# slbouknight/accelerated-ray-tracer

Measured on AMD Instinct MI355X. Metric: Mrays/s, 1200x800 random scene @ 500 spp (frame ms in ms_per_step), higher is better.
Workload: dtype f32

## Files before the change

### accelerated-ray-tracer_amd/csrc/rt_abi.hip

```cpp
#include <hip/hip_runtime.h>

#include <algorithm>
#include <cfloat>
#include <utility>
#include <cmath>
#include <functional>
#include <cstdio>
#include <cstring>
#include <string>
#include <vector>

#include "../../include/rt_abi.h"
#include "rt_device.h"
#include "rt_refit_host.h"

namespace {

struct device_info {
    bool ready = false;
    int num_cu = 256;
    size_t lds_per_cu = 160 * 1024;
};
enum { RT_MAX_DEVICES = 16 };
device_info g_devices[RT_MAX_DEVICES];
// ... 2223 lines not shown
            HIPCHK(hipMemcpy((void*)*v.dev, v.host, list_bytes, hipMemcpyHostToDevice));
        }
        HIPCHK(mem.get((void**)&mp.out, list_bytes));
        HIPCHK(hipMemset(mp.out, 0xFF, list_bytes));
    }
    HIPCHK(rt_launch_math_tests(mp, nullptr));
    HIPCHK(hipDeviceSynchronize());
    if (sweep) HIPCHK(hipMemcpy(digests, mp.digests, n_digests * sizeof(unsigned long long), hipMemcpyDeviceToHost));
    else HIPCHK(hipMemcpy(out, mp.out, list_bytes, hipMemcpyDeviceToHost));
    return RT_OK;
}

rt_status rt_debug_cal_cost(rt_scene* s, uint32_t* out, int32_t cap, int32_t* nx, int32_t* ny) {
    if (!s) return invalid("rt_debug_cal_cost: null scene");
    if (!out || !nx || !ny) return invalid("rt_debug_cal_cost: null argument");
    if (cap < 64) return invalid("rt_debug_cal_cost: cap must be at least 64 (the smallest calibration grid is 8 x 8)");
    if (!s->d_cal_cost || s->cal_nx <= 0 || s->cal_ny <= 0) return invalid("rt_debug_cal_cost: the scene kept no calibration costs");
    *nx = s->cal_nx; *ny = s->cal_ny;
    if ((long long)cap < (long long)s->cal_nx * s->cal_ny) return invalid("rt_debug_cal_cost: cap is smaller than the calibration grid (nx and ny are set)");
    RT_TRY(use_device(s->device));
    HIPCHK(hipMemcpy(out, s->d_cal_cost, (size_t)s->cal_nx * s->cal_ny * sizeof(unsigned int), hipMemcpyDeviceToHost));
    return RT_OK;
}

rt_status rt_debug_cost_map(rt_scene* s, uint32_t* out, int64_t cap, int32_t* info4) {
    if (!s) return invalid("rt_debug_cost_map: null scene");
    if (!info4 || (!out && cap != 0)) return invalid("rt_debug_cost_map: null argument");
    RT_TRY(use_device(s->device));
    if (s->frame_pending) RT_TRY(rt_frame_finish(s, nullptr));
    const rt_scene::cost_map_state& cm = s->cost_map;
    const bool have = g_opt.cost_map && cm.valid;
    info4[0] = !have ? 0 : (cm.scene_epoch == s->scene_epoch && cm.opt_epoch == g_opt_epoch ? 1 : 2);
    info4[1] = have ? cm.key.nx : 0; info4[2] = have ? cm.key.local_rows : 0; info4[3] = cm.last_parts;
    if (!have || !out) return RT_OK;
    const long long n = (long long)cm.key.nx * cm.key.local_rows;
    if ((long long)cap < n) return invalid("rt_debug_cost_map: cap is smaller than the map (info is set)");
    HIPCHK(hipMemcpy(out, cm.d, (size_t)n * sizeof(unsigned int), hipMemcpyDeviceToHost));
    return RT_OK;
}

rt_status rt_debug_set_cost_map(rt_scene* s, const uint32_t* in, int64_t n) {
    if (!s) return invalid("rt_debug_set_cost_map: null scene");
    if (!in) return invalid("rt_debug_set_cost_map: null argument");
    if (!g_opt.cost_map) return invalid("rt_debug_set_cost_map: option cost_map is 0");
    rt_scene::cost_map_state& cm = s->cost_map;
    if (!cm.have_last_key) return invalid("rt_debug_set_cost_map: the scene has rendered no ranked frame");
    if ((long long)n != (long long)cm.last_key.nx * cm.last_key.local_rows) return invalid("rt_debug_set_cost_map: n is not the last ranked frame's local pixel count");
    RT_TRY(use_device(s->device));
    if (s->frame_pending) RT_TRY(rt_frame_finish(s, nullptr));
    std::vector<unsigned int> words((size_t)n);
    unsigned long long total = 0;
    for (size_t k = 0; k < (size_t)n; ++k) { words[k] = in[k] & 0x7FFFFFFFu; total += words[k]; }
    cm.valid = false;
    RT_TRY(grow(cm.d, cm.capacity, (size_t)n));
    HIPCHK(hipMemcpy(cm.d, words.data(), (size_t)n * sizeof(unsigned int), hipMemcpyHostToDevice));
    cm.key = cm.last_key; cm.scene_epoch = s->scene_epoch; cm.opt_epoch = g_opt_epoch; cm.total = total; cm.valid = true;
    return RT_OK;
}

rt_status rt_debug_rank_info(rt_scene* s, uint32_t* out13) {
    if (!s) return invalid("rt_debug_rank_info: null scene");
    if (!out13) return invalid("rt_debug_rank_info: null argument");
    if (!s->ranked_frame || !s->d_rank) return invalid("rt_debug_rank_info: the scene's last frame was not ranked");
    RT_TRY(use_device(s->device));
    if (s->frame_pending) HIPCHK(hipStreamSynchronize(s->pending_stream));
    HIPCHK(hipMemcpy(out13, s->d_rank, sizeof(rt_rank_info), hipMemcpyDeviceToHost));
    return RT_OK;
}

namespace {
struct main_launch {
    int kernel, lds_mode;
    size_t lds_bytes;
    dim3 grid, block;
    int per_cu_resident;
    bool lean_family;
};
rt_status plan_main_launch(const rt_scene* s, int kernel, size_t n_pixels, rt_frame_params& fp, main_launch& ml) {
    const int g_num_cu = g_devices[s->device].num_cu;
    const size_t g_lds_per_cu = g_devices[s->device].lds_per_cu;
    int lds_mode = g_opt.lds_mode;
    const bool lean_family = s->spheres_only && s->tex_level < 2;
    const size_t budget1 = g_lds_per_cu - 2048;
    if (lds_mode < 0) {
        if (s->node_bytes + s->sphere_bytes <= budget1) lds_mode = 2;
        else if (s->node_bytes <= budget1) lds_mode = 1;
        else lds_mode = 0;
    }
    if (g_opt.lds_mode < 0 && kernel == RT_KERNEL_STAGED && g_opt.scan_nodes > 0 && s->dev.n_nodes <= g_opt.scan_nodes) lds_mode = 4;
    if (lds_mode >= 3 && kernel != RT_KERNEL_STAGED) lds_mode = 2;
    if (kernel == RT_KERNEL_PIXEL) lds_mode = 0;
    size_t lds_bytes = 0;
    if (lds_mode >= 1 && lds_mode <= 3) lds_bytes += s->node_bytes;
    if (lds_mode >= 2 && lds_mode <= 3) lds_bytes += s->sphere_bytes;
    if (lds_mode == 3) lds_bytes += s->shade_bytes;
    if (lds_bytes > budget1) return invalid("requested lds_mode does not fit the CU's LDS");
    dim3 grid, block;
    int per_cu_resident = 1;
    if (kernel == RT_KERNEL_PIXEL) {
        block = dim3(256);
        grid = dim3((fp.work_items + 255u) / 256u);
    } else {
        const bool lean = lean_family;
        const int fam_max_threads = lean ? RT_LEAN_MAX_THREADS : RT_HEAVY_MAX_THREADS;
        const int lds_fit = lds_bytes ? (int)(g_lds_per_cu / (lds_bytes + 512)) : 8;
        int per_cu = g_opt.wg_per_cu > 0 ? g_opt.wg_per_cu : (lean ? 2 : 3);
        int threads = g_opt.threads > 0 ? g_opt.threads : (lean ? 512 : 256);
        if (g_opt.wg_per_cu <= 0 && g_opt.threads <= 0 && lds_fit < per_cu) {
            per_cu = 1; threads = fam_max_threads;
        }
        if (lds_fit < per_cu) per_cu = lds_fit < 1 ? 1 : lds_fit;
        if (threads > fam_max_threads) threads = fam_max_threads;
        if (threads < 64) threads = 64;
        block = dim3((unsigned)threads);
        unsigned want = (unsigned)(g_num_cu * per_cu);
        const unsigned need = (fp.work_items + (unsigned)threads - 1) / (unsigned)threads;
        grid = dim3(want < need ? want : need);
        per_cu_resident = per_cu;
    }
    {
        const double pixels_per_lane = (double)n_pixels / ((double)g_num_cu * (double)per_cu_resident * (double)block.x);
        const bool latency_regime = kernel == RT_KERNEL_STAGED && lean_family && pixels_per_lane < 2.75;
        fp.shade_threshold = g_opt.shade_threshold > 0 ? g_opt.shade_threshold : (latency_regime ? 16 : 32);
        fp.newpath_threshold = g_opt.newpath_threshold > 0 ? g_opt.newpath_threshold : (s->spheres_only ? (latency_regime ? 12 : 24) : 8);
    }
    ml.kernel = kernel; ml.lds_mode = lds_mode; ml.lds_bytes = lds_bytes; ml.grid = grid; ml.block = block; ml.per_cu_resident = per_cu_resident;
    ml.lean_family = lean_family;
    return RT_OK;
}

void stats_of_launch(const rt_scene* s, const main_launch& ml, rt_stats& out) {
    out.kernel_variant = ml.kernel * 1000 + ml.lds_mode * 100 + s->tex_level * 10 + (s->spheres_only ? 1 : 0);
    out.workgroups = (int)ml.grid.x; out.threads_per_group = (int)ml.block.x; out.lds_bytes = (int)ml.lds_bytes;
}

void fill_frame_params(const rt_scene* s, const rt_frame_desc* f, const frame_geometry& g, int ns, rt_frame_params& fp) {
    memset(&fp, 0, sizeof(fp));
    fp.ray_counter = s->d_ray_counter;
    fp.work_counter = s->d_work_counter;
    fp.seed_base = f->seed_base;
    fp.nx = f->nx; fp.ny = f->ny; fp.ns = ns; fp.gamma = f->gamma;
    fp.background[0] = f->background[0]; fp.background[1] = f->background[1]; fp.background[2] = f->background[2];
    fp.use_gradient_bg = f->use_gradient_bg;
    fp.tile_rows = f->tile_rows; fp.tile_first = f->tile_first; fp.tile_stride = f->tile_stride;
    fp.local_rows = g.local_rows;
    fp.tiles_x = g.tiles_x;
    fp.work_items = g.work_items;
    fp.sparse_priority = g_opt.sparse_priority; fp.sparse_eager = g_opt.sparse_eager; fp.semi_priority = g_opt.semi_priority; fp.tier_priority = g_opt.tier_priority;
    fp.steps_per_trip = g_opt.steps_per_trip;
    fp.leaf_threshold = g_opt.leaf_threshold;
    fp.diel_threshold = g_opt.diel_threshold;
    fp.box_threshold = g_opt.box_threshold; fp.medium_threshold = g_opt.medium_threshold;
}

struct tier_room {
    bool fits;
    int lds_scene;
    size_t lds;
    unsigned tail_grid;
};
tier_room plan_tier_room(const rt_scene* s, size_t budget) {
    tier_room r = {false, 0, 0, 0};
    const int ns_ = s->dev.n_slots, nsph = s->dev.n_spheres, nm = s->dev.n_materials, nt = s->dev.n_textures;
    if (s->dev.leaf_lo == nullptr || rt_tier_lds_bytes(ns_, nsph, nm, nt, false) > budget) return r;
    r.fits = true;
    r.lds_scene = rt_tier_lds_bytes(ns_, nsph, nm, nt, true) <= budget ? 1 : 0;
    r.lds = rt_tier_lds_bytes(ns_, nsph, nm, nt, r.lds_scene != 0);
    const bool lean_family = s->spheres_only && s->tex_level < 2;
    const unsigned by_lds = (unsigned)(g_devices[s->device].lds_per_cu / (r.lds + 512));
    const unsigned by_regs = lean_family ? 4u : 3u;
    r.tail_grid = (unsigned)g_devices[s->device].num_cu * (by_lds < by_regs ? by_lds : by_regs);
    if (r.tail_grid < 1u) r.tail_grid = 1u;
    return r;
}
hipError_t launch_tier(const rt_scene* s, const rt_frame_params& fp, dim3 grid, size_t lds, hipStream_t stream) {
    return s->spheres_only ? rt_launch_tier_spheres(s->tex_level, s->dev, fp, grid, lds, stream)
// ... 540 lines not shown
```

### accelerated-ray-tracer_amd/csrc/rt_device.h

```cpp
#pragma once
#include <hip/hip_runtime.h>
#include <stdint.h>

#include "../../include/rt_abi.h"

#define RT_PERSISTENT_THREADS 512
#ifndef RT_LEAN_MIN_WAVES
#define RT_LEAN_MIN_WAVES 4
#endif
#ifndef RT_LEAN_MAX_THREADS
#define RT_LEAN_MAX_THREADS 512
#endif
#define RT_HEAVY_MAX_THREADS 768
#define RT_HEAVY_MIN_WAVES 3

#define RT_TIER_THREADS 256
enum { RT_DIAG_BINS = 192, RT_DIAG_T0_SLOT = 32, RT_DIAG_HIST_SLOT = 33, RT_DIAG_WAVE_SLOT = 33 + 2 * 192 + 7, RT_DIAG_MAX_WAVES = 8192,
       RT_COUNTER_BYTES = (33 + 2 * 192 + 7 + 2 * 8192) * 8 };
enum { RT_KERNEL_PIXEL = 0, RT_KERNEL_STAGED = 3 };

struct rt_pixel_state {
    uint32_t rng[6];
    float col[3];
    uint32_t cost;
};

struct rt_rank_info {
    uint32_t heavy_items;
    uint32_t heavy_threshold;
    uint32_t tier1_items;
    uint32_t tier2_items;
    int32_t tier1_wgs;
    int32_t main_skip_wgs;
    int32_t sparse_wgs;
    int32_t sparse_stride;
    int32_t semi_wgs;
    int32_t semi_stride;
    uint32_t threshold1;
    uint32_t threshold2;
    uint32_t collected;
};

struct rt_rank_params {
    rt_pixel_state* state;
    const unsigned int* tile_cost;
    unsigned int* tile_order;
    const unsigned long long* ray_counter;
    unsigned long long* heavy_list;
    unsigned int* heavy_pixels;
    rt_rank_info* info;
    uint32_t n_pixels, n_tiles, heavy_cap;
    uint32_t max_grid, waves_per_wg, normal_need;
    int32_t sparse_stride;
    int32_t semi_stride;
    int32_t sparse_percent;
    int32_t sparse_work_percent;
    int32_t tier_possible;
    int32_t tier1_pixels;
    int32_t tier1_depth;
    int32_t tier_wgs_cap;
    int32_t tier_waves_per_main_wg;
    int32_t nx, smooth_percent;
    float heavy_factor, sparse_factor, tier1_factor;
};

#define RT_NODE_SKIP(stored) (~(stored))

struct rt_scene_dev {
    const rt_node* nodes;
    const rt_node* nodes_ref;
    const rt_sphere* spheres;
    const rt_quad* quads;
    const rt_box* boxes;
    const rt_instance* instances;
    const rt_medium* media;
    const rt_material* materials;
    const rt_texture* textures;
    const uint8_t* images;
    int32_t n_nodes, n_nodes_ref, n_spheres, n_materials, n_textures;
    float bound[3];
    float bound_pad;
    const float4* leaf_lo;
    const float4* leaf_hi;
    const float* slot_ranges;
    int32_t n_leaves, n_slots;
    int32_t n_media_leaves;
    int32_t media_ord[2];
    rt_camera camera;
};

enum { RT_WC_DEAD = 64,
       RT_WC_PUSHED = 65,
       RT_WC_TAIL_HEAD = 66,
       RT_WORK_COUNTER_BYTES = 512 };
struct rt_frame_params {
    float* fb;
    unsigned long long* ray_counter;
    unsigned int* work_counter;
    unsigned int* pixel_cost;
    unsigned int* node_pass;
    int32_t node_pass_lds;
    float* ray_sample;
    uint32_t ray_sample_cap, ray_sample_stride;
    const unsigned int* tile_order;
    unsigned int* tile_cost;
    rt_pixel_state* state_out;
    const rt_pixel_state* state_in;
    int32_t sample_begin, sample_end;
    const unsigned int* heavy_pixels;
    const rt_rank_info* rank;
    int32_t store_parked;
    int32_t fresh;
    int32_t tier_lds_scene;
    unsigned long long* handoff_queue;
    uint32_t handoff_cap;
    rt_pixel_state* handoff_state;
    int32_t handoff_pixels;
    int32_t handoff_poll_ticks;
    int32_t tail_mode;
    unsigned int* cost_out;
    uint64_t seed_base;
    int32_t nx, ny, ns;
    float gamma;
    float background[3];
    int32_t use_gradient_bg;
    int32_t tile_rows, tile_first, tile_stride;
    int32_t local_rows;
    int32_t tiles_x;
    uint32_t work_items;
    int32_t sparse_eager;
    int32_t sparse_priority;
    int32_t tier_priority;
    int32_t semi_priority;
    int32_t steps_per_trip;
    int32_t shade_threshold;
    int32_t leaf_threshold;
    int32_t box_threshold, medium_threshold;
    int32_t diel_threshold;
    int32_t newpath_threshold;
};

hipError_t rt_launch_rank(const rt_rank_params& rp, hipStream_t st);
struct rt_prior_params {
    rt_pixel_state* state;
    unsigned int* tile_cost;
    unsigned long long* total;
    const unsigned int* cal_cost;
    int32_t cal_nx, cal_ny;
    int32_t nx, ny, local_rows, tiles_x;
// ... 286 lines not shown
```

### accelerated-ray-tracer_amd/csrc/rt_device_funcs.h

```cpp
#pragma once
#include <hip/hip_runtime.h>
#include <float.h>
#include <stdint.h>

#include "../../include/rt_abi.h"
#include "rt_device.h"
#include "rt_xorwow.h"

#define DEV __device__ __forceinline__

namespace {

struct f3 { float x, y, z; };
DEV f3 mk3(float x, float y, float z) { f3 r; r.x = x; r.y = y; r.z = z; return r; }
DEV f3 ld3(const float* p) { return mk3(p[0], p[1], p[2]); }
DEV f3 operator+(f3 a, f3 b) { return mk3(a.x + b.x, a.y + b.y, a.z + b.z); }
DEV f3 operator-(f3 a, f3 b) { return mk3(a.x - b.x, a.y - b.y, a.z - b.z); }
DEV f3 operator*(f3 a, f3 b) { return mk3(a.x * b.x, a.y * b.y, a.z * b.z); }
DEV f3 operator*(float t, f3 v) { return mk3(t * v.x, t * v.y, t * v.z); }
DEV f3 operator-(f3 a) { return mk3(-a.x, -a.y, -a.z); }
DEV f3 sdiv(f3 v, float t) { return mk3(v.x / t, v.y / t, v.z / t); }
DEV float dot(f3 a, f3 b) { return fmaf(a.z, b.z, fmaf(a.x, b.x, a.y * b.y)); }
DEV f3 cross(f3 a, f3 b) { return mk3(fmaf(a.y, b.z, -(a.z * b.y)), -fmaf(a.x, b.z, -(a.z * b.x)), fmaf(a.x, b.y, -(a.y * b.x))); }
DEV float length(f3 v) { return sqrtf(fmaf(v.z, v.z, fmaf(v.x, v.x, v.y * v.y))); }
// ... 454 lines not shown
        out.d = random_in_unit_sphere(g);
        attenuation = (TEX > 0 && m.tex >= 0) ? texture_value<TEX>(sc, m.tex, rec.u, rec.v, rec.p) : ld3(m.albedo);
        return true;
    }
    }
}

DEV Ray camera_get_ray(const rt_camera& c, float s, float t, rt_xorwow& g) {
    f3 p;
    do {
        const float a = rt_xorwow_signed(g);
        const float b = rt_xorwow_signed(g);
        p = mk3(a, b, 0.0f);
    } while (dot(p, p) >= 1.0f);
    const f3 rd = c.lens_radius * p;
    const f3 cu = ld3(c.u), cv = ld3(c.v);
    const f3 offset = fma3(rd.x, cu, rd.y * cv);
    const double tm = fma((double)rt_xorwow_uniform(g), c.time1 - c.time0, c.time0);
    const f3 origin = ld3(c.origin);
    Ray r;
    r.o = origin + offset;
    r.d = (fma3(t, ld3(c.vertical), fma3(s, ld3(c.horizontal), ld3(c.lower_left_corner))) - origin) - offset;
    r.tm = (float)tm;
    return r;
}

DEV float apply_gamma(float c, float gamma) {
    if (gamma == 1.0f) return c;
    const float inv = 1.0f / gamma;
    return cr_pow(fmaxf(c, 0.0f), inv);
}

template <typename P>
DEV f3 miss_color(const P& fp, const Ray& r) {
    f3 bg = mk3(fp.background[0], fp.background[1], fp.background[2]);
    if (fp.use_gradient_bg) {
        const f3 ud = unit_vector(r.d);
        const float t = 0.5f * (ud.y + 1.0f);
        bg = mk3(fmaf(t, 0.5f, 1.0f - t), fmaf(t, 0.7f, 1.0f - t), (1.0f - t) + t);
    }
    return bg;
}

DEV bool work_to_pixel(const rt_frame_params& fp, uint32_t w, int& i, int& lrow) {
    const uint32_t tile = fp.tile_order ? fp.tile_order[w >> 6] : (w >> 6), within = w & 63u;
    const uint32_t tx = tile % (uint32_t)fp.tiles_x, ty = tile / (uint32_t)fp.tiles_x;
    i = (int)(tx * 8u + (within & 7u));
    lrow = (int)(ty * 8u + (within >> 3));
    return i < fp.nx && lrow < fp.local_rows;
}
DEV int local_to_global_row(const rt_frame_params& fp, int lrow) {
    const int t = lrow / fp.tile_rows;
    return (fp.tile_first + t * fp.tile_stride) * fp.tile_rows + (lrow - t * fp.tile_rows);
}

DEV void store_pixel(const rt_frame_params& fp, int i, int lrow, f3 col) {
    const float k = (float)(1.0 / (double)(float)fp.ns);
    col = mk3(col.x * k, col.y * k, col.z * k);
    float* px = fp.fb + ((size_t)lrow * fp.nx + i) * 3;
    px[0] = apply_gamma(col.x, fp.gamma);
    px[1] = apply_gamma(col.y, fp.gamma);
    px[2] = apply_gamma(col.z, fp.gamma);
}

typedef float lds_native_float4 __attribute__((ext_vector_type(4)));
DEV int32_t lds_address(const void* p) { return (int32_t)(uint32_t)(uintptr_t)(const __attribute__((address_space(3))) void*)p; }
DEV float4 lds_load_float4(int32_t address, int which) {
    const lds_native_float4 q = ((const __attribute__((address_space(3))) lds_native_float4*)(uintptr_t)(uint32_t)address)[which];
    return make_float4(q.x, q.y, q.z, q.w);
}
DEV int32_t lds_load_word(int32_t address, int word) { return ((const __attribute__((address_space(3))) int32_t*)(uintptr_t)(uint32_t)address)[word]; }

template <int LDS_MODE, bool WALK_LINKS = false>
DEV SceneView stage_scene(const rt_scene_dev& sd, unsigned char* lds) {
    SceneView v;
    v.nodes = sd.nodes; v.spheres = sd.spheres; v.quads = sd.quads; v.boxes = sd.boxes; v.instances = sd.instances;
    v.media = sd.media; v.materials = sd.materials; v.textures = sd.textures; v.images = sd.images; v.n_nodes = sd.n_nodes;
    if (LDS_MODE >= 1 && LDS_MODE <= 3) {
        float4* dst = reinterpret_cast<float4*>(lds);
        const float4* src = reinterpret_cast<const float4*>(sd.nodes);
        const int n16 = sd.n_nodes * 2;
        if (WALK_LINKS) {
            const int32_t base = lds_address(lds);
            for (int k = threadIdx.x; k < n16; k += blockDim.x) {
                float4 q = src[k];
                const int32_t w = __float_as_int(q.w);
                q.w = __int_as_float(w < 0 ? base + 32 * RT_NODE_SKIP(w) : ~w);
                dst[k] = q;
            }
        } else {
            for (int k = threadIdx.x; k < n16; k += blockDim.x) dst[k] = src[k];
        }
        v.nodes = reinterpret_cast<const rt_node*>(lds);
        if (LDS_MODE >= 2) {
            float4* dst2 = dst + n16;
            const float4* src2 = reinterpret_cast<const float4*>(sd.spheres);
            const int m16 = sd.n_spheres * 2;
            for (int k = threadIdx.x; k < m16; k += blockDim.x) dst2[k] = src2[k];
            v.spheres = reinterpret_cast<const rt_sphere*>(dst2);
            if (LDS_MODE >= 3) {
                float4* dst3 = dst2 + m16;
                const float4* src3 = reinterpret_cast<const float4*>(sd.materials);
                const int q16 = sd.n_materials * 2;
                for (int k = threadIdx.x; k < q16; k += blockDim.x) dst3[k] = src3[k];
                v.materials = reinterpret_cast<const rt_material*>(dst3);
                float4* dst4 = dst3 + q16;
                const float4* src4 = reinterpret_cast<const float4*>(sd.textures);
                const int r16 = sd.n_textures * 4;
                for (int k = threadIdx.x; k < r16; k += blockDim.x) dst4[k] = src4[k];
                v.textures = reinterpret_cast<const rt_texture*>(dst4);
            }
        }
        __syncthreads();
    }
    return v;
}

template <bool SPHERES_ONLY>
DEV bool trace(const SceneView& sc, const Ray& r, HitInfo& best, unsigned int* pass_count = nullptr) {
    const f3 inv = mk3(1.0f / r.d.x, 1.0f / r.d.y, 1.0f / r.d.z);
    const float tmin = 0.001f;
    best.t = FLT_MAX; best.prim = -1; best.inst = -1;
    const float4* nodes4 = reinterpret_cast<const float4*>(sc.nodes);
    int i = 0;
    const int n = sc.n_nodes;
    while (i < n) {
        const float4 a = nodes4[2 * i], b = nodes4[2 * i + 1];
        int next = RT_NODE_SKIP(__float_as_int(a.w));
        if (slab_test(a, b, r.o, inv, tmin, best.t)) {
            if (pass_count) atomicAdd(&pass_count[i], 1u);
            const int32_t prim = __float_as_int(b.w);
            if (prim >= 0) leaf_test<SPHERES_ONLY>(sc, prim, r, tmin, best);
            else next = i + 1;
        }
        i = next;
    }
    return best.prim >= 0;
}

DEV bool inv_is_finite(const f3 inv) {
    return fabsf(inv.x) < INFINITY && fabsf(inv.y) < INFINITY && fabsf(inv.z) < INFINITY;
}

DEV void slab_interval(const float4 lo_skip, const float4 hi_prim, const f3 o, const f3 inv, float tmin, float& t_enter, float& t_exit) {
    float tmax = FLT_MAX;
    float t0 = (lo_skip.x - o.x) * inv.x, t1 = (hi_prim.x - o.x) * inv.x;
    if (inv.x < 0.0f) { const float tmp = t0; t0 = t1; t1 = tmp; }
    tmin = t0 > tmin ? t0 : tmin;
    tmax = t1 < tmax ? t1 : tmax;
    t0 = (lo_skip.y - o.y) * inv.y; t1 = (hi_prim.y - o.y) * inv.y;
    if (inv.y < 0.0f) { const float tmp = t0; t0 = t1; t1 = tmp; }
    tmin = t0 > tmin ? t0 : tmin;
    tmax = t1 < tmax ? t1 : tmax;
    t0 = (lo_skip.z - o.z) * inv.z; t1 = (hi_prim.z - o.z) * inv.z;
    if (inv.z < 0.0f) { const float tmp = t0; t0 = t1; t1 = tmp; }
    tmin = t0 > tmin ? t0 : tmin;
    tmax = t1 < tmax ? t1 : tmax;
    t_enter = tmin; t_exit = tmax;
}

DEV bool lane_not(bool b) { return __builtin_amdgcn_inverse_ballot_w64(~__builtin_amdgcn_ballot_w64(b)); }

DEV bool slab_interval_open(float tmin, float tmax, float x0, float x1, float y0, float y1, float z0, float z1) {
    float lo = __builtin_amdgcn_fmed3f(tmin, x0, x1), hi = __builtin_amdgcn_fmed3f(tmax, x0, x1);
    lo = __builtin_amdgcn_fmed3f(lo, y0, y1); hi = __builtin_amdgcn_fmed3f(hi, y0, y1);
    lo = __builtin_amdgcn_fmed3f(lo, z0, z1); hi = __builtin_amdgcn_fmed3f(hi, z0, z1);
    return !(hi <= lo);
}

DEV bool slab_test_finite(const float4 lo_skip, const float4 hi_prim, const f3 o, const f3 inv, float tmin, float tmax) {
    const float x0 = (lo_skip.x - o.x) * inv.x, x1 = (hi_prim.x - o.x) * inv.x;
    const float y0 = (lo_skip.y - o.y) * inv.y, y1 = (hi_prim.y - o.y) * inv.y;
    const float z0 = (lo_skip.z - o.z) * inv.z, z1 = (hi_prim.z - o.z) * inv.z;
    return slab_interval_open(tmin, tmax, x0, x1, y0, y1, z0, z1);
}

struct LooseRay { f3 clo, chi; };
DEV bool loose_ok(const f3 inv, const f3 o, const float* bound) {
// ... 21 lines not shown
```

### accelerated-ray-tracer_amd/csrc/rt_kernel_staged.h

```cpp
#pragma once
#ifndef RT_STEP_UNROLL
#define RT_STEP_UNROLL 2
#endif
#include "rt_device_funcs.h"
#include "rt_launch.h"

#ifdef RT_DIAG
#define DIAG_ADD(slot, value) do { const unsigned long long v_ = (unsigned long long)(value); if ((threadIdx.x & 63) == 0) diag_local[slot] += v_; } while (0)
#define DIAG_T(slot) do { const unsigned long long n_ = __builtin_readcyclecounter(); diag_time[slot] += n_ - diag_t_last; diag_t_last = n_; } while (0)
#else
#define DIAG_ADD(slot, value) do { } while (0)
#define DIAG_T(slot) do { } while (0)
#endif

template <bool SPHERES_ONLY, int TEX, bool NEED_UV, int LDS_MODE>
__global__ void __launch_bounds__((SPHERES_ONLY && TEX < 2) ? RT_LEAN_MAX_THREADS : RT_HEAVY_MAX_THREADS, (SPHERES_ONLY && TEX < 2) ? RT_LEAN_MIN_WAVES : RT_HEAVY_MIN_WAVES) rt_render_staged_kernel(rt_scene_dev sd, rt_frame_params fp) {
    extern __shared__ __attribute__((aligned(16))) unsigned char lds[];
#ifdef RT_DIAG
    unsigned long long diag_local[16] = {0, 0, 0, 0, 0, 0, 0, 0, 0, 0, 0, 0, 0, 0, 0, 0};
    unsigned long long diag_time[8] = {0, 0, 0, 0, 0, 0, 0, 0};
    unsigned long long diag_shade_cycles = 0;
    unsigned long long diag_t_last = 0;
    const unsigned long long diag_t_start = __builtin_amdgcn_s_memrealtime();
    if ((threadIdx.x & 63) == 0) atomicMin(fp.ray_counter + RT_DIAG_T0_SLOT, diag_t_start);
    unsigned long long diag_fetch_t = 0ull, diag_done_t = 0ull;
    unsigned int diag_last_px = 0u, diag_last_src = 0u;
#endif
    constexpr bool SCAN = LDS_MODE == 4;
    rt_rank_info rk;
    rk.heavy_items = 0u; rk.heavy_threshold = 0xFFFFFFFFu; rk.tier1_items = 0u; rk.tier2_items = 0u;
    rk.tier1_wgs = 0; rk.main_skip_wgs = 0; rk.sparse_wgs = 0; rk.sparse_stride = 1; rk.semi_wgs = 0; rk.semi_stride = 1;
    if (fp.rank) {
        const rt_rank_info* q = fp.rank;
        rk.heavy_items = q->heavy_items; rk.heavy_threshold = q->heavy_threshold; rk.tier1_items = q->tier1_items;
        rk.tier2_items = q->tier2_items; rk.semi_wgs = q->semi_wgs; rk.semi_stride = q->semi_stride;
        rk.main_skip_wgs = q->main_skip_wgs; rk.sparse_wgs = q->sparse_wgs; rk.sparse_stride = q->sparse_stride;
    }
    const int wg = (int)blockIdx.x - rk.main_skip_wgs;
    if (wg < 0) return;
    constexpr bool ADDR = LDS_MODE >= 1 && LDS_MODE <= 3;
    const SceneView sc = stage_scene<LDS_MODE, ADDR>(sd, lds);
    const float4* nodes4 = reinterpret_cast<const float4*>(sc.nodes);
    const int n_nodes = sc.n_nodes;
    const int root = ADDR ? lds_address(lds) : 0;
    const int limit = ADDR ? __builtin_amdgcn_readfirstlane(root + 32 * n_nodes) : n_nodes;
    const int ST_DONE = limit, ST_NEWPATH = limit + 1, ST_DIEL = limit + 2, ST_SETUP = limit + 3, ST_DEAD = limit + 4;
    auto node_lo = [&](int at) -> float4 { return ADDR ? lds_load_float4(at, 0) : nodes4[2 * at]; };
    auto node_hi = [&](int at) -> float4 { return ADDR ? lds_load_float4(at, 1) : nodes4[2 * at + 1]; };
    auto leaf_prim = [](const float4 hi) -> int32_t { return ADDR ? ~__float_as_int(hi.w) : __float_as_int(hi.w); };
    const float tmin = 0.001f;

    rt_xorwow g = {0, 0, 0, 0, 0, 0};
    int px_i = 0, px_lrow = 0, px_j = 0, sample = 0, bounce = 0;
    f3 col = mk3(0, 0, 0), throughput = mk3(1, 1, 1), radiance = mk3(0, 0, 0);
    Ray cur; cur.o = mk3(0, 0, 0); cur.d = mk3(0, 0, 1); cur.tm = 0.f;
    f3 inv = mk3(1, 1, 1);
    HitInfo best; best.t = FLT_MAX; best.prim = -1; best.inst = -1;
    int node = ST_NEWPATH;
    int32_t parked = -1;
    int32_t pend = -1;
    float cur_a = 1.f;
    bool have_pixel = false, first = true, finite_inv = true;
    bool tier3_open = true;
    bool leave = false;
    unsigned int wave_dead = 0;
    unsigned long long last_poll = 0ull;
    bool dry_seen = false;
    const uint32_t total_lanes = (uint32_t)((int)gridDim.x - rk.main_skip_wgs) * blockDim.x;
    unsigned int rays = 0, rays_at_pixel_start = 0;
    bool sparse = wg < rk.sparse_wgs;
    bool semi = !sparse && wg < rk.sparse_wgs + rk.semi_wgs;
#ifdef RT_DIAG
    const bool diag_was_sparse = sparse;
#endif
    if (semi && fp.semi_priority > 0) {
        if (fp.semi_priority == 1) __builtin_amdgcn_s_setprio(1);
        else if (fp.semi_priority == 2) __builtin_amdgcn_s_setprio(2);
        else __builtin_amdgcn_s_setprio(3);
    }
    if (sparse && fp.sparse_priority > 0) {
        if (fp.sparse_priority == 1) __builtin_amdgcn_s_setprio(1);
        else if (fp.sparse_priority == 2) __builtin_amdgcn_s_setprio(2);
        else __builtin_amdgcn_s_setprio(3);
    }

#ifdef RT_DIAG
    diag_t_last = __builtin_readcyclecounter();
#endif
    for (;;) {
        DIAG_ADD(0, 1);
        DIAG_T(7);
        if (SCAN) {
            const bool scanning = (unsigned)node < (unsigned)n_nodes;
            if (__ballot(scanning) != 0ull) {
                const bool ref_form = __ballot(scanning && !finite_inv) != 0ull;
                int resume = 0;
                for (int k = 0; k < n_nodes; ++k) {
                    const float4 a = uniform_load(nodes4 + 2 * k), b = uniform_load(nodes4 + 2 * k + 1);
                    const int32_t prim = __builtin_amdgcn_readfirstlane(__float_as_int(b.w));
                    const int skip = RT_NODE_SKIP(__builtin_amdgcn_readfirstlane(__float_as_int(a.w)));
                    const bool active = scanning && k >= resume;
                    DIAG_ADD(1, 1); DIAG_ADD(2, __popcll(__ballot(active)));
                    const bool pass = active && (ref_form ? slab_test(a, b, cur.o, inv, tmin, best.t) : slab_test_finite(a, b, cur.o, inv, tmin, best.t));
                    if (prim < 0) {
                        if (active && !pass) resume = skip;
                        DIAG_T(0);
                    } else if (__ballot(pass) != 0ull) {
                        DIAG_T(0);
                        DIAG_ADD(3, 1); DIAG_ADD(4, __popcll(__ballot(pass)));
                        if (pass) leaf_test<SPHERES_ONLY, true>(sc, prim, cur, tmin, best);
                        DIAG_T(1);
                    }
                }
                if (scanning) node = ST_DONE;
            }
        } else {
        if (__ballot(!finite_inv && (unsigned)node < (unsigned)limit) == 0ull) {
            const int trip_pairs = ((sparse ? 2 * fp.steps_per_trip : fp.steps_per_trip) + RT_STEP_UNROLL - 1) / RT_STEP_UNROLL;
            const LooseRay lr = loose_setup(inv, cur.o, sd.bound);
            for (int pair = 0; pair < trip_pairs; ++pair) {
                if (__ballot((unsigned)node < (unsigned)limit) == 0ull) break;
#pragma unroll
                for (int half = 0; half < RT_STEP_UNROLL; ++half) {
                    DIAG_ADD(1, 1); DIAG_ADD(2, __popcll(__ballot((unsigned)node < (unsigned)limit)));
                    if ((unsigned)node < (unsigned)limit) {
                        const float4 a = node_lo(node), b = node_hi(node);
                        const bool pass = slab_test_loose(a, b, inv, lr, tmin, best.t);
                        if (ADDR) {
                            const int32_t link = __float_as_int(b.w), skip = __float_as_int(a.w);
                            const bool is_leaf = link < 0, noted = pend >= 0;
                            const bool inner = lane_not(is_leaf), clear = lane_not(noted);
                            const bool at_leaf = pass && is_leaf;
                            const bool stop = at_leaf && noted;
                            pend = (at_leaf && clear) ? node : pend;
                            parked = stop ? node : parked;
                            node = (pass && (inner || noted)) ? link : skip;
                        } else {
                            const int32_t link = __float_as_int(b.w), nskip = __float_as_int(a.w);
                            const bool is_leaf = link >= 0, noted = pend >= 0;
                            const bool inner = lane_not(is_leaf), clear = lane_not(noted);
                            const bool at_leaf = pass && is_leaf;
                            const bool stop = at_leaf && noted;
                            const int next = ~((pass && inner) ? link : nskip);
                            pend = (at_leaf && clear) ? node : pend;
                            parked = stop ? node : parked;
                            node = stop ? nskip : next;
                        }
                    }
                }
            }
        } else {
            for (int step = 0; step < fp.steps_per_trip; ++step) {
                if (__ballot((unsigned)node < (unsigned)limit) == 0ull) break;
                if ((unsigned)node < (unsigned)limit) {
                    const float4 a = node_lo(node), b = node_hi(node);
                    const bool pass = slab_test(a, b, cur.o, inv, tmin, best.t);
                    if (ADDR) {
                        const int32_t link = __float_as_int(b.w), skip = __float_as_int(a.w);
                        const bool at_leaf = pass && link < 0;
                        const bool stop = at_leaf && (pend >= 0 || !finite_inv);
                        pend = (at_leaf && !stop) ? node : pend;
                        parked = stop ? node : parked;
                        node = (pass && (link >= 0 || stop)) ? link : skip;
                    } else {
                        const int32_t link = __float_as_int(b.w), nskip = __float_as_int(a.w);
                        const bool at_leaf = pass && link >= 0;
                        const bool stop = at_leaf && (pend >= 0 || !finite_inv);
                        const int next = ~((pass && link < 0) ? link : nskip);
                        pend = (at_leaf && !stop) ? node : pend;
                        parked = stop ? node : parked;
                        node = stop ? nskip : next;
                    }
                }
            }
        }
        DIAG_T(0);
        for (;;) {
            const int cand = pend >= 0 ? pend : (node < 0 ? parked : -1);
            const unsigned long long due_mask = __ballot(cand >= 0);
            const bool nobody_steps = __ballot((unsigned)node < (unsigned)limit) == 0ull;
            const int live_b = __popcll(__ballot(node != ST_DEAD));
            if (due_mask != 0ull && (nobody_steps || sparse || __popcll(due_mask) >= 1 + ((fp.leaf_threshold - 1) * live_b >> 6))) {
                DIAG_ADD(3, 1); DIAG_ADD(4, __popcll(due_mask));
                int kind = -1;
                int32_t prim = -1;
                bool box_ok = false;
                if (cand >= 0) {
                    const float4 a = node_lo(cand), b = node_hi(cand);
                    prim = leaf_prim(b);
                    kind = SPHERES_ONLY ? RT_PRIM_SPHERE : RT_PRIM_KIND(prim);
                    box_ok = finite_inv ? slab_test_finite(a, b, cur.o, inv, tmin, best.t) : true;
                }
                bool tested = false;
                if (SPHERES_ONLY) {
                    if (cand >= 0) {
                        float t;
                        if (box_ok && sphere_test_a(sc.spheres[RT_PRIM_INDEX(prim)], cur, cur_a, tmin, best.t, t)) { best.t = t; best.prim = prim; best.inst = -1; }
                        tested = true;
                    }
                } else {
                    if (kind == RT_PRIM_SPHERE || kind == RT_PRIM_QUAD) {
                        float t;
                        const bool hit = box_ok && (kind == RT_PRIM_SPHERE ? sphere_test_a(sc.spheres[RT_PRIM_INDEX(prim)], cur, cur_a, tmin, best.t, t)
                                                                           : quad_test(sc.quads[RT_PRIM_INDEX(prim)], cur, tmin, best.t, t));
                        if (hit) { best.t = t; best.prim = prim; best.inst = -1; }
                        tested = true;
                    }
                    const unsigned long long box_mask = __ballot(kind == RT_PRIM_BOX || kind == RT_PRIM_INSTANCE);
                    if (box_mask != 0ull && (nobody_steps || __popcll(box_mask) >= 1 + ((fp.box_threshold - 1) * live_b >> 6))) {
                        if (kind == RT_PRIM_BOX || kind == RT_PRIM_INSTANCE) {
                            float t;
                            int32_t leaf = prim, inst = -1;
                            if (box_ok && solid_test(sc, prim, cur, tmin, best.t, t, leaf, inst)) { best.t = t; best.prim = leaf; best.inst = inst; }
                            tested = true;
                        }
                    }
                    const unsigned long long med_mask = __ballot(kind == RT_PRIM_MEDIUM);
                    if (med_mask != 0ull && (nobody_steps || __popcll(med_mask) >= 1 + ((fp.medium_threshold - 1) * live_b >> 6))) {
                        if (kind == RT_PRIM_MEDIUM) {
                            float t;
                            if (box_ok && medium_test(sc, sc.media[RT_PRIM_INDEX(prim)], cur, tmin, best.t, t)) { best.t = t; best.prim = prim; best.inst = -1; }
                            tested = true;
                        }
                    }
                }
                if (tested) {
                    if (node < 0) {
                        node = ADDR ? lds_load_word(parked, 3) : ~node;
                        pend = pend >= 0 ? parked : -1; parked = -1;
                    }
                    else pend = -1;
                }
                if (nobody_steps && __ballot((unsigned)node < (unsigned)limit) == 0ull && __ballot(pend >= 0 || node < 0) != 0ull) continue;
            }
            break;
        }
        }
        DIAG_T(1);
        if (node == ST_DONE && pend < 0 && best.prim < 0) {
            radiance = fma3(throughput, miss_color(fp, cur), radiance);
            node = ST_NEWPATH;
        }
        const unsigned long long walking = __ballot(node < limit);
        const bool force = walking == 0ull;
        const int n_done = __popcll(__ballot(node == ST_DONE && pend < 0));
        bool ran_stage = false;
        const int live = __popcll(__ballot(node != ST_DEAD));
        const int shade_need = 1 + ((fp.shade_threshold - 1) * live >> 6);
        const int diel_need = 1 + ((fp.diel_threshold - 1) * live >> 6);
        const int newpath_need = 1 + ((fp.newpath_threshold - 1) * live >> 6);
        const bool eager = sparse && fp.sparse_eager;

        DIAG_T(6);
        if (n_done > 0 && (n_done >= shade_need || force || eager)) {
            ran_stage = true;
            DIAG_ADD(5, 1); DIAG_ADD(6, n_done);
            DIAG_ADD(11, __popcll(__ballot(node == ST_DONE && pend < 0 && best.prim >= 0)));
            if (node == ST_DONE && pend < 0) {
                {
                    const HitRec rec = resolve_hit<SPHERES_ONLY, NEED_UV>(sc, cur, best);
                    const rt_material m = sc.materials[rec.mat];
                    if (m.kind == RT_MAT_DIELECTRIC) {
                        if (sparse) {
                            const f3 dir = dielectric_direction(cur.d, rec.n, m.ior, g);
                            ++bounce;
                            if (bounce >= 50) node = ST_NEWPATH;
                            else { cur.o = rec.p; cur.d = dir; node = ST_SETUP; }
                        } else {
                            node = ST_DIEL;
                        }
                    } else if (m.kind == RT_MAT_DIFFUSE_LIGHT) {
                        const f3 emitted = (TEX > 0 && m.tex >= 0) ? texture_value<TEX>(sc, m.tex, rec.u, rec.v, rec.p) : ld3(m.albedo);
                        radiance = fma3(throughput, emitted, radiance);
                        node = ST_NEWPATH;
                    } else {
                        const f3 rs = random_in_unit_sphere(g);
                        f3 dir, attenuation;
                        bool go_on = true;
                        if (m.kind == RT_MAT_METAL) {
                            const f3 reflected = reflect(unit_vector(cur.d), rec.n);
                            dir = fma3(m.fuzz, rs, reflected);
                            attenuation = ld3(m.albedo);
                            go_on = dot(dir, rec.n) > 0.0f;
                        } else {
                            if (m.kind == RT_MAT_LAMBERTIAN) {
                                const f3 target = (rec.p + rec.n) + rs;
                                dir = target - rec.p;
                            } else {
                                dir = rs;
                            }
                            attenuation = (TEX > 0 && m.tex >= 0) ? texture_value<TEX>(sc, m.tex, rec.u, rec.v, rec.p) : ld3(m.albedo);
                        }
                        ++bounce;
                        if (!go_on || bounce >= 50) node = ST_NEWPATH;
                        else {
                            throughput = throughput * attenuation;
                            cur.o = rec.p; cur.d = dir;
                            node = ST_SETUP;
                        }
                    }
                }
            }
        }
        DIAG_T(2);
        {
            const int n_diel = __popcll(__ballot(node == ST_DIEL));
            if (n_diel > 0 && (n_diel >= diel_need || force || eager)) {
                ran_stage = true;
                DIAG_ADD(7, 1); DIAG_ADD(8, n_diel);
                if (node == ST_DIEL) {
                    const HitRec rec = resolve_hit<SPHERES_ONLY, false>(sc, cur, best);
                    const f3 dir = dielectric_direction(cur.d, rec.n, sc.materials[rec.mat].ior, g);
// ... 177 lines not shown
```

Baseline: 14150.

## Encode leaf self-address in LDS link word and add separate leaf-primitive table

In the LDS address-walk mode, leaf nodes now store the bitwise-complemented LDS address of the node itself instead of the primitive index, and a separate per-node primitive table is staged into LDS after the nodes. This lets the traversal loop drop the 'parked' register bookkeeping and simplifies the per-step select logic, since the stopped leaf is recovered as ~node. The cost is extra LDS footprint (4 bytes per node), which can reduce occupancy or push scenes into a lower lds_mode, plus an extra LDS load per leaf test.

```diff
diff --git a/accelerated-ray-tracer_amd/csrc/rt_abi.hip b/accelerated-ray-tracer_amd/csrc/rt_abi.hip
--- a/accelerated-ray-tracer_amd/csrc/rt_abi.hip
+++ b/accelerated-ray-tracer_amd/csrc/rt_abi.hip
@@ -2329,16 +2329,17 @@
     int lds_mode = g_opt.lds_mode;
     const bool lean_family = s->spheres_only && s->tex_level < 2;
     const size_t budget1 = g_lds_per_cu - 2048;
+    const size_t image_bytes = s->node_bytes + (kernel == RT_KERNEL_STAGED ? (size_t)RT_WALK_PRIM_TABLE_BYTES(s->dev.n_nodes) : 0);
     if (lds_mode < 0) {
-        if (s->node_bytes + s->sphere_bytes <= budget1) lds_mode = 2;
-        else if (s->node_bytes <= budget1) lds_mode = 1;
+        if (image_bytes + s->sphere_bytes <= budget1) lds_mode = 2;
+        else if (image_bytes <= budget1) lds_mode = 1;
         else lds_mode = 0;
     }
     if (g_opt.lds_mode < 0 && kernel == RT_KERNEL_STAGED && g_opt.scan_nodes > 0 && s->dev.n_nodes <= g_opt.scan_nodes) lds_mode = 4;
     if (lds_mode >= 3 && kernel != RT_KERNEL_STAGED) lds_mode = 2;
     if (kernel == RT_KERNEL_PIXEL) lds_mode = 0;
     size_t lds_bytes = 0;
-    if (lds_mode >= 1 && lds_mode <= 3) lds_bytes += s->node_bytes;
+    if (lds_mode >= 1 && lds_mode <= 3) lds_bytes += image_bytes;
     if (lds_mode >= 2 && lds_mode <= 3) lds_bytes += s->sphere_bytes;
     if (lds_mode == 3) lds_bytes += s->shade_bytes;
     if (lds_bytes > budget1) return invalid("requested lds_mode does not fit the CU's LDS");
diff --git a/accelerated-ray-tracer_amd/csrc/rt_device.h b/accelerated-ray-tracer_amd/csrc/rt_device.h
--- a/accelerated-ray-tracer_amd/csrc/rt_device.h
+++ b/accelerated-ray-tracer_amd/csrc/rt_device.h
@@ -65,6 +65,7 @@
 };
 
 #define RT_NODE_SKIP(stored) (~(stored))
+#define RT_WALK_PRIM_TABLE_BYTES(n_nodes) ((4 * (n_nodes) + 15) & ~15)
 
 struct rt_scene_dev {
     const rt_node* nodes;
diff --git a/accelerated-ray-tracer_amd/csrc/rt_device_funcs.h b/accelerated-ray-tracer_amd/csrc/rt_device_funcs.h
--- a/accelerated-ray-tracer_amd/csrc/rt_device_funcs.h
+++ b/accelerated-ray-tracer_amd/csrc/rt_device_funcs.h
@@ -560,18 +560,20 @@
         const int n16 = sd.n_nodes * 2;
         if (WALK_LINKS) {
             const int32_t base = lds_address(lds);
+            int32_t* prim_of = reinterpret_cast<int32_t*>(dst + n16);
             for (int k = threadIdx.x; k < n16; k += blockDim.x) {
                 float4 q = src[k];
                 const int32_t w = __float_as_int(q.w);
-                q.w = __int_as_float(w < 0 ? base + 32 * RT_NODE_SKIP(w) : ~w);
+                q.w = __int_as_float(w < 0 ? base + 32 * RT_NODE_SKIP(w) : ~(base + 16 * (k - 1)));
                 dst[k] = q;
+                if (k & 1) prim_of[k >> 1] = w;
             }
         } else {
             for (int k = threadIdx.x; k < n16; k += blockDim.x) dst[k] = src[k];
         }
         v.nodes = reinterpret_cast<const rt_node*>(lds);
         if (LDS_MODE >= 2) {
-            float4* dst2 = dst + n16;
+            float4* dst2 = dst + n16 + (WALK_LINKS ? RT_WALK_PRIM_TABLE_BYTES(sd.n_nodes) / 16 : 0);
             const float4* src2 = reinterpret_cast<const float4*>(sd.spheres);
             const int m16 = sd.n_spheres * 2;
             for (int k = threadIdx.x; k < m16; k += blockDim.x) dst2[k] = src2[k];
diff --git a/accelerated-ray-tracer_amd/csrc/rt_kernel_staged.h b/accelerated-ray-tracer_amd/csrc/rt_kernel_staged.h
--- a/accelerated-ray-tracer_amd/csrc/rt_kernel_staged.h
+++ b/accelerated-ray-tracer_amd/csrc/rt_kernel_staged.h
@@ -47,7 +47,8 @@
     const int ST_DONE = limit, ST_NEWPATH = limit + 1, ST_DIEL = limit + 2, ST_SETUP = limit + 3, ST_DEAD = limit + 4;
     auto node_lo = [&](int at) -> float4 { return ADDR ? lds_load_float4(at, 0) : nodes4[2 * at]; };
     auto node_hi = [&](int at) -> float4 { return ADDR ? lds_load_float4(at, 1) : nodes4[2 * at + 1]; };
-    auto leaf_prim = [](const float4 hi) -> int32_t { return ADDR ? ~__float_as_int(hi.w) : __float_as_int(hi.w); };
+    const int prim_of = ADDR ? limit - (root >> 3) : 0;
+    auto leaf_prim = [&](int at, const float4 hi) -> int32_t { return ADDR ? lds_load_word(prim_of + (at >> 3), 0) : __float_as_int(hi.w); };
     const float tmin = 0.001f;
 
     rt_xorwow g = {0, 0, 0, 0, 0, 0};
@@ -128,13 +129,10 @@
                         const bool pass = slab_test_loose(a, b, inv, lr, tmin, best.t);
                         if (ADDR) {
                             const int32_t link = __float_as_int(b.w), skip = __float_as_int(a.w);
-                            const bool is_leaf = link < 0, noted = pend >= 0;
-                            const bool inner = lane_not(is_leaf), clear = lane_not(noted);
-                            const bool at_leaf = pass && is_leaf;
-                            const bool stop = at_leaf && noted;
-                            pend = (at_leaf && clear) ? node : pend;
-                            parked = stop ? node : parked;
-                            node = (pass && (inner || noted)) ? link : skip;
+                            const bool inner = link >= 0, noted = pend >= 0;
+                            const bool take = pass & (inner | noted);
+                            pend = (pass != take) ? node : pend;
+                            node = take ? link : skip;
                         } else {
                             const int32_t link = __float_as_int(b.w), nskip = __float_as_int(a.w);
                             const bool is_leaf = link >= 0, noted = pend >= 0;
@@ -160,7 +158,6 @@
                         const bool at_leaf = pass && link < 0;
                         const bool stop = at_leaf && (pend >= 0 || !finite_inv);
                         pend = (at_leaf && !stop) ? node : pend;
-                        parked = stop ? node : parked;
                         node = (pass && (link >= 0 || stop)) ? link : skip;
                     } else {
                         const int32_t link = __float_as_int(b.w), nskip = __float_as_int(a.w);
@@ -176,7 +173,8 @@
         }
         DIAG_T(0);
         for (;;) {
-            const int cand = pend >= 0 ? pend : (node < 0 ? parked : -1);
+            const int32_t stopped_at = ADDR ? ~node : parked;
+            const int cand = pend >= 0 ? pend : (node < 0 ? stopped_at : -1);
             const unsigned long long due_mask = __ballot(cand >= 0);
             const bool nobody_steps = __ballot((unsigned)node < (unsigned)limit) == 0ull;
             const int live_b = __popcll(__ballot(node != ST_DEAD));
@@ -187,7 +185,7 @@
                 bool box_ok = false;
                 if (cand >= 0) {
                     const float4 a = node_lo(cand), b = node_hi(cand);
-                    prim = leaf_prim(b);
+                    prim = leaf_prim(cand, b);
                     kind = SPHERES_ONLY ? RT_PRIM_SPHERE : RT_PRIM_KIND(prim);
                     box_ok = finite_inv ? slab_test_finite(a, b, cur.o, inv, tmin, best.t) : true;
                 }
@@ -226,8 +224,8 @@
                 }
                 if (tested) {
                     if (node < 0) {
-                        node = ADDR ? lds_load_word(parked, 3) : ~node;
-                        pend = pend >= 0 ? parked : -1; parked = -1;
+                        node = ADDR ? lds_load_word(stopped_at, 3) : ~node;
+                        pend = pend >= 0 ? stopped_at : -1; parked = -1;
                     }
                     else pend = -1;
                 }
```

Measured after the change: 14470, median of 6. 2.2% higher.
